# h33p/ofps

Measured on AMD Instinct MI355X. Metric: Mvectors/s, 1080p 16x16 blocks +-16 full-search SAD, higher is better.
Workload: dtype u8

## Files before the change

ofps_amd/csrc/sad.hip:

```cpp
#include "common.hpp"

#include <cstdlib>
#include <utility>

namespace {

constexpr int kWavesPerWG = 4;

constexpr int pick_stride(int min_s, int k, int ng) {
    for (int s = min_s; s < min_s + 64; ++s)
        if ((k * s) % 32 == ng % 32) return s;
    return min_s | 1;
}

template <int B, int R, int K>
struct SadCfg {
    static_assert(B % 4 == 0 && R % 4 == 0, "tile origin must stay dword aligned");
    static_assert(B * B * 255 <= 65535, "packed u16 SAD accumulators would overflow");
    static constexpr int NCAND = 2 * R + 1;
    static constexpr int NG = (NCAND + 3) / 4;
    static constexpr int NC = (NCAND + K - 1) / K;
    static constexpr int T = NG * NC;
    static constexpr int PASSES = (T + 63) / 64;
    static constexpr int BW = B / 4;
// ... 226 lines not shown
    asm volatile("" : "+v"(base));
    (strip_row<B, R, I0, RR>(acc, c, lds, base), ...);
}

#ifndef OFPS_SAD_COLKEYS
#define OFPS_SAD_COLKEYS 2
#endif
constexpr int kSadColKeys = OFPS_SAD_COLKEYS;
constexpr int kColSlotDwords = kSadColKeys == 2 ? 4 * 64 : 0;

template <int B, int R, int I0>
__device__ __forceinline__ void strip_pass(const uint32_t (&c)[B][B / 4], const uint32_t* lds, uint32_t tile_off,
                                           const uint32_t (&colk)[4], const uint32_t (&colk_pos)[4], int y0, int H, uint32_t& bkey, int& bi,
                                           uint32_t (&colmin)[4], uint32_t* amin) {
    using C = StripCfg<B, R>;
    unsigned long long acc[C::NP];
#pragma unroll
    for (int ii = 0; ii < C::NP; ++ii) acc[ii] = 0;
    constexpr int ROWS = ((I0 + C::NP < C::NCAND ? C::NP : C::NCAND - I0) + B - 1);
    strip_rows<B, R, I0>(acc, c, lds, tile_off, std::make_integer_sequence<int, ROWS>{});
#pragma unroll
    for (int ii = 0; ii < C::NP; ++ii) asm volatile("" : "+v"(acc[ii]));
    if constexpr (kSadColKeys != 0 && (C::RANK_KEY || C::COMPACT_KEY)) {
        auto low_of = [&](int ii) -> uint32_t {
            const int i = I0 + ii, dy = -R + i;
            const bool ok = i < C::NCAND && y0 + dy >= 0 && y0 + dy + B <= H;
            return ok ? (uint32_t)(C::RANK_KEY ? ((dy * dy) << 1 | (dy > 0 ? 1 : 0)) : ((dy * dy) << 6 | i)) : 0xFFFFFFFFu;
        };
        uint32_t hmask = 0xFFFF0000u;
        asm volatile("" : "+v"(hmask));
        auto keys_of = [&](int ii, uint32_t low, uint32_t (&k)[4]) {
            const uint32_t lo = (uint32_t)acc[ii], hi = (uint32_t)(acc[ii] >> 32);
            k[0] = (lo << 16) | low; k[1] = (lo & hmask) | low; k[2] = (hi << 16) | low; k[3] = (hi & hmask) | low;
        };
        if constexpr (kSadColKeys == 1) {
#pragma unroll
            for (int ii = 0; ii < C::NP; ii += 2) {
                if (I0 + ii >= C::NCAND) break;
                uint32_t ka[4], kb[4];
                keys_of(ii, low_of(ii), ka);
                if (ii + 1 < C::NP && I0 + ii + 1 < C::NCAND) {
                    keys_of(ii + 1, low_of(ii + 1), kb);
#pragma unroll
                    for (int j = 0; j < 4; ++j)
                        asm("v_min3_u32 %0, %1, %2, %3" : "=v"(colmin[j]) : "v"(colmin[j]), "v"(ka[j]), "v"(kb[j]));
                } else {
#pragma unroll
                    for (int j = 0; j < 4; ++j) colmin[j] = min(colmin[j], ka[j]);
                }
            }
        } else {
#pragma unroll
            for (int ii = 0; ii < C::NP; ++ii) {
                if (I0 + ii >= C::NCAND) break;
                uint32_t k[4];
                keys_of(ii, low_of(ii), k);
#pragma unroll
                for (int j = 0; j < 4; ++j) __hip_atomic_fetch_min(amin + 64 * j, k[j], __ATOMIC_RELAXED, __HIP_MEMORY_SCOPE_WAVEFRONT);
            }
        }
        return;
    }
#pragma unroll
    for (int ii = 0; ii < C::NP; ++ii) {
        const int i = I0 + ii;
        const int dy = -R + i;
        if (i < C::NCAND && y0 + dy >= 0 && y0 + dy + B <= H) {
            const uint32_t lo = (uint32_t)acc[ii], hi = (uint32_t)(acc[ii] >> 32);
            const uint32_t (&ck)[4] = (C::RANK_KEY && dy > 0) ? colk_pos : colk;
            const uint32_t k0 = (lo << 16) | ck[0];
            const uint32_t k1 = (lo & 0xFFFF0000u) | ck[1];
            const uint32_t k2 = (hi << 16) | ck[2];
            const uint32_t k3 = (hi & 0xFFFF0000u) | ck[3];
            if constexpr (C::RANK_KEY) {
                bkey = min(bkey, __builtin_elementwise_add_sat(min(min(k0, k1), min(k2, k3)), (uint32_t)((dy * dy) << 3)));
            } else if constexpr (C::COMPACT_KEY) {
                const uint32_t m = __builtin_elementwise_add_sat(min(min(k0, k1), min(k2, k3)), (uint32_t)((dy * dy) << 6 | i));
                bkey = min(bkey, m);
            } else {
                const uint32_t m = __builtin_elementwise_add_sat(min(min(k0, k1), min(k2, k3)), (uint32_t)(dy * dy));
                const bool lt = m < bkey;
                bkey = lt ? m : bkey;
                bi = lt ? i : bi;
            }
        }
    }
}

template <int B, int R, int... S>
__device__ __forceinline__ void strip_passes(const uint32_t (&c)[B][B / 4], const uint32_t* lds, uint32_t tile_off,
                                             const uint32_t (&colk)[4], const uint32_t (&colk_pos)[4], int y0, int H, uint32_t& bkey, int& bi,
                                             uint32_t (&colmin)[4], uint32_t* amin, std::integer_sequence<int, S...>) {
    (strip_pass<B, R, S * StripCfg<B, R>::NP>(c, lds, tile_off, colk, colk_pos, y0, H, bkey, bi, colmin, amin), ...);
}

constexpr int kStripWaves = 4;

template <int B, int R>
__device__ __forceinline__ void strip_body(const SadParams& p, int strips_per_row, int strip, uint32_t* tiles, int wave, int lane) {
    using C = StripCfg<B, R>;
    const int strips_per_pair = strips_per_row * p.nby;
    const int pair = (int)div48((unsigned)strip, p.div_spp);
    const int rem = strip - pair * strips_per_pair;
    const int by = (int)div48((unsigned)rem, p.div_spr);
    const int bx0 = (rem - by * strips_per_row) * C::NB;

    const uint8_t* __restrict__ prev = p.prev_base + (size_t)pair * p.prev_pitch;
    const uint8_t* __restrict__ cur = p.cur_base + (size_t)pair * p.cur_pitch;
    uint32_t* tile = tiles + wave * C::TILE_DWORDS;

    const int b = lane / C::NG;
    const int g = lane % C::NG;
    const int bx = bx0 + b;
    const bool blk_on = bx < p.nbx;
    const int y0 = by * B;

    uint32_t c[B][C::BW];
    {
        const int bxc = blk_on ? bx : p.nbx - 1;
        const uint8_t* cp = cur + (size_t)y0 * p.stride + bxc * B;
#pragma unroll
        for (int y = 0; y < B; ++y) {
            if constexpr (C::BW % 4 == 0) {
#pragma unroll
                for (int q4 = 0; q4 < C::BW; q4 += 4) {
                    const uint4 v = *reinterpret_cast<const uint4*>(cp + (size_t)y * p.stride + 4 * q4);
                    c[y][q4 + 0] = v.x; c[y][q4 + 1] = v.y; c[y][q4 + 2] = v.z; c[y][q4 + 3] = v.w;
                }
            } else {
#pragma unroll
                for (int q2 = 0; q2 < C::BW; q2 += 2) {
                    const uint2 v = *reinterpret_cast<const uint2*>(cp + (size_t)y * p.stride + 4 * q2);
                    c[y][q2 + 0] = v.x; c[y][q2 + 1] = v.y;
                }
            }
        }
    }

    {
        constexpr int LR = 64 / C::TILE_WG;
        constexpr int STEPS = (C::TILE_H + LR - 1) / LR;
        const int tx0 = bx0 * B - R, ty0 = y0 - R;
        const int sr = lane / C::TILE_WG, sc = lane - sr * C::TILE_WG;
        const int gx = tx0 + C::GRAN * sc;
        const bool lane_on = sr < LR && gx >= 0 && gx < p.W;
        const uint8_t* src = prev + (ptrdiff_t)(ty0 + sr) * p.stride + gx;
        uint32_t* dst = tile + sr * C::SW + C::GDW * sc;
#pragma unroll
        for (int it = 0; it < STEPS; ++it) {
            const int row = sr + it * LR;
            const bool row_in_tile = (it + 1) * LR <= C::TILE_H || row < C::TILE_H;
            if (lane_on && row_in_tile && (unsigned)(ty0 + row) < (unsigned)p.H) {
                const uint8_t* sp = src + (ptrdiff_t)(it * LR) * p.stride;
                uint32_t* dp = dst + it * LR * C::SW;
                if constexpr (C::GRAN == 16) *reinterpret_cast<uint4*>(dp) = *reinterpret_cast<const uint4*>(sp);
                else if constexpr (C::GRAN == 8) *reinterpret_cast<uint2*>(dp) = *reinterpret_cast<const uint2*>(sp);
                else *dp = *reinterpret_cast<const uint32_t*>(sp);
            }
        }
    }
    __builtin_amdgcn_fence(__ATOMIC_RELEASE, "wavefront");
    __builtin_amdgcn_wave_barrier();
    __builtin_amdgcn_fence(__ATOMIC_ACQUIRE, "wavefront");

    const int dx0 = -R + 4 * g;
    uint32_t colk[4], colk_pos[4];
#pragma unroll
    for (int j = 0; j < 4; ++j) {
        const int dx = dx0 + j;
        const int x = bx * B + dx;
        const bool v = blk_on && g < C::NGA && x >= 0 && x + B <= p.W;
        const uint32_t rank = dx0 < 0 ? 3u - j : (uint32_t)j;
        colk[j] = v ? ((uint32_t)(dx * dx) << C::KSHIFT) | (C::RANK_KEY ? rank : 0u) : 0xFFFFFFFFu;
        colk_pos[j] = v ? ((uint32_t)(dx * dx) << C::KSHIFT) | (7u - rank) : 0xFFFFFFFFu;
    }
    uint32_t bkey = 0xFFFFFFFFu;
    int bi = 0;
    uint32_t colmin[4] = {0xFFFFFFFFu, 0xFFFFFFFFu, 0xFFFFFFFFu, 0xFFFFFFFFu};
    uint32_t* amin = nullptr;
    if constexpr (kSadColKeys == 2 && (C::RANK_KEY || C::COMPACT_KEY)) {
        amin = tiles + kStripWaves * C::TILE_DWORDS + wave * kColSlotDwords + lane;
#pragma unroll
        for (int j = 0; j < 4; ++j) amin[64 * j] = 0xFFFFFFFFu;
    }
    strip_passes<B, R>(c, tiles, (uint32_t)(wave * C::TILE_DWORDS + b * C::BW + g), colk, colk_pos, y0, p.H, bkey, bi, colmin, amin,
                       std::make_integer_sequence<int, C::SPLIT>{});
    if constexpr (kSadColKeys != 0 && (C::RANK_KEY || C::COMPACT_KEY)) {
#pragma unroll
        for (int j = 0; j < 4; ++j) {
            uint32_t kc;
            if constexpr (kSadColKeys == 2) kc = __hip_atomic_load(amin + 64 * j, __ATOMIC_RELAXED, __HIP_MEMORY_SCOPE_WAVEFRONT);
            else kc = colmin[j];
            uint32_t lk;
            if constexpr (C::RANK_KEY) {
                const uint32_t x = (((kc & 0xFFFEu) << 2) + colk[j]) ^ ((kc & 1u) * 7u);
                lk = (kc & 0xFFFF0000u) | x;
            } else {
                lk = (kc & 0xFFFF0000u) | ((kc & 0xFFFFu) + colk[j]);
            }
            lk = (colk[j] == 0xFFFFFFFFu || kc == 0xFFFFFFFFu) ? 0xFFFFFFFFu : lk;
            bkey = min(bkey, lk);
        }
    }
    unsigned long long best = ~0ull;
    if (bkey != 0xFFFFFFFFu) {
        const uint32_t d2 = (bkey & 0xFFFFu) >> C::KSHIFT;
        int dx = dx0, dy;
        if constexpr (C::RANK_KEY) {
            const int code = (int)(bkey & 7u);
            const bool neg = code < 4;
            const int rank = neg ? code : 7 - code;
            dx = dx0 + (dx0 < 0 ? 3 - rank : rank);
            const int ady = (int)(__builtin_sqrtf((float)((int)d2 - dx * dx)) + 0.5f);
            dy = neg ? -ady : ady;
        } else {
            if constexpr (C::COMPACT_KEY) bi = (int)(bkey & 63u);
            dy = -R + bi;
            const int dxsq = (int)d2 - dy * dy;
#pragma unroll
            for (int j = 1; j < 4; ++j) dx = ((dx0 + j) * (dx0 + j) == dxsq) ? dx0 + j : dx;
        }
        best = ((unsigned long long)((bkey & 0xFFFF0000u) | d2) << 32) | (unsigned long long)(uint32_t)(((dy + R) << 8) | (dx + R));
    }
    uint32_t eacc[C::KE];
#pragma unroll
    for (int i = 0; i < C::KE; ++i) eacc[i] = 0;
    {
        const uint32_t* ecol = tile + b * C::BW + C::EDGE_COL;
        const int erow0 = g * C::KE;
        uint32_t nxt[C::BW];
#pragma unroll
        for (int q = 0; q < C::BW; ++q) nxt[q] = ecol[erow0 * C::SW + q];
#pragma unroll
        for (int rr = 0; rr < B + C::KE - 1; ++rr) {
            uint32_t ref[C::BW];
#pragma unroll
            for (int q = 0; q < C::BW; ++q) ref[q] = nxt[q];
            if (rr + 1 < B + C::KE - 1) {
                const int row = erow0 + rr + 1;
#pragma unroll
                for (int q = 0; q < C::BW; ++q) nxt[q] = ecol[row * C::SW + q];
            }
#pragma unroll
            for (int i = 0; i < C::KE; ++i) {
                const int y = rr - i;
                if (y >= 0 && y < B) {
#pragma unroll
                    for (int q = 0; q < C::BW; ++q) eacc[i] = __builtin_amdgcn_sad_u8(ref[q], c[y][q], eacc[i]);
                }
            }
            asm volatile("" : "+v"(eacc[0]) : : "memory");
        }
    }

    {
        const bool xok = blk_on && bx * B + R + B <= p.W;
#pragma unroll
        for (int i = 0; i < C::KE; ++i) {
            const int dy = -R + g * C::KE + i;
            const bool v = xok && dy <= R && y0 + dy >= 0 && y0 + dy + B <= p.H;
            const unsigned long long k64 =
                ((unsigned long long)((eacc[i] << 16) | (uint32_t)(R * R + dy * dy)) << 32) |
                (unsigned long long)(uint32_t)(((dy + R) << 8) | (2 * R));
            best = (v && k64 < best) ? k64 : best;
        }
    }
#pragma unroll
    for (int m = 1; m < C::NG; m <<= 1) {
        const unsigned long long o = shfl_xor_u64(best, m);
        best = o < best ? o : best;
    }
    if (blk_on && g == 0) {
        const int sad = (int)(best >> 48);
        const int dy = (int)((best >> 8) & 0xFF) - R, dx = (int)(best & 0xFF) - R;
        const size_t k = ((size_t)pair * p.nby + by) * p.nbx + bx;
        float4 e;
        e.x = (float)(bx * B + B / 2 + dx) * p.nx;
        e.y = (float)(y0 + B / 2 + dy) * p.ny;
        e.z = ((float)dx / 1.0f) * (-p.nx);
        e.w = ((float)dy / 1.0f) * (-p.ny);
        p.out_entries[k] = e;
        if (p.out_best) {
            p.out_best[3 * k + 0] = dx;
            p.out_best[3 * k + 1] = dy;
            p.out_best[3 * k + 2] = sad;
        }
    }
}

template <int B, int R>
__global__ __launch_bounds__(64 * kStripWaves, (StripCfg<B, R>::MIN_WAVES)) void sad_strip_kernel(const SadParams p, int strips_per_row,
                                                                      int total_strips) {
    using C = StripCfg<B, R>;
    __shared__ __attribute__((aligned(16))) uint32_t tiles[kStripWaves * (C::TILE_DWORDS + kColSlotDwords)];
    const int wave = __builtin_amdgcn_readfirstlane(threadIdx.x >> 6);
    const int lane = threadIdx.x & 63;
    const int per_xcd = gridDim.x / 8;
    const int lwg = (int)(blockIdx.x % 8) * per_xcd + (int)(blockIdx.x / 8);
    const int strip = lwg * kStripWaves + wave;
    if (strip >= total_strips) return;
    strip_body<B, R>(p, strips_per_row, strip, tiles, wave, lane);
}

template <int B, int R>
__global__ __launch_bounds__(64 * kStripWaves, (StripCfg<B, R>::MIN_WAVES)) void sad_strip_list_kernel(const SadParams p, int strips_per_row,
                                                                           const uint32_t* __restrict__ strip_list) {
    using C = StripCfg<B, R>;
    __shared__ __attribute__((aligned(16))) uint32_t tiles[kStripWaves * (C::TILE_DWORDS + kColSlotDwords)];
    const int wave = __builtin_amdgcn_readfirstlane(threadIdx.x >> 6);
    const int lane = threadIdx.x & 63;
    const int count = (int)strip_list[0];
#pragma unroll 1
    for (int k = (int)blockIdx.x * kStripWaves + wave; k < count; k += (int)gridDim.x * kStripWaves)
        strip_body<B, R>(p, strips_per_row, (int)strip_list[1 + k], tiles, wave, lane);
}

struct PdeCfg {
    static constexpr int B = 16, R = 16, STEP = 4, PR = B / STEP;
    using C = StripCfg<B, R>;
    static constexpr int CUR_DW = B * C::NB * C::BW;
    static constexpr int CAP = 512;
    static constexpr int WAVE_DW = C::TILE_DWORDS + 4 + CUR_DW + CAP + 2 * C::NB;
    static constexpr int OFF_CUR = C::TILE_DWORDS + 4, OFF_LIST = OFF_CUR + CUR_DW, OFF_BEST = OFF_LIST + CAP;
    static_assert(OFF_BEST % 2 == 0, "64-bit keys must be 8-byte aligned");
};

template <int RR>
__device__ __forceinline__ void pde_row(unsigned long long (&acc)[PdeCfg::C::NP], const uint32_t (&c)[PdeCfg::PR][PdeCfg::C::BW],
                                        const uint32_t* lds, uint32_t& base) {
    using C = PdeCfg::C;
    constexpr int B = PdeCfg::B, R = PdeCfg::R, STEP = PdeCfg::STEP;
    constexpr int G = StripWalk<B, R>::ROWS_PER_BASE;
    if constexpr (RR > 0 && RR % G == 0) {
        base += G * C::SW;
        asm volatile("" : "+v"(base));
    }
    unsigned long long win[C::BW];
#pragma unroll
    for (int q = 0; q < C::BW; ++q) win[q] = reinterpret_cast<const U64A4*>(lds + base + (RR % G) * C::SW + q)->v;
#pragma unroll
    for (int ii = 0; ii < C::NP; ++ii) {
        const int y = RR - ii;
        if (ii < C::NCAND && y >= 0 && y < B && y % STEP == 0) {
#pragma unroll
            for (int q = 0; q < C::BW; ++q) acc[ii] = __builtin_amdgcn_qsad_pk_u16_u8(win[q], c[y / STEP][q], acc[ii]);
        }
    }
}
template <int... RR>
__device__ __forceinline__ void pde_rows(unsigned long long (&acc)[PdeCfg::C::NP], const uint32_t (&c)[PdeCfg::PR][PdeCfg::C::BW],
                                         const uint32_t* lds, uint32_t tile_off, std::integer_sequence<int, RR...>) {
    uint32_t base = tile_off;
    asm volatile("" : "+v"(base));
    (pde_row<RR>(acc, c, lds, base), ...);
}

__device__ __forceinline__ uint32_t pde_two_rows(const uint32_t* tile, const uint32_t* curl, int bb, int dyi, int dxi, int r8) {
    using C = PdeCfg::C;
    const int sh = dxi & 3;
    uint32_t s = 0;
#pragma unroll
    for (int k = 0; k < 2; ++k) {
        const int y = 2 * r8 + k;
        const uint32_t* rp = tile + (dyi + y) * C::SW + bb * C::BW + (dxi >> 2);
        const uint32_t* cp = curl + y * (C::NB * C::BW) + bb * C::BW;
        uint32_t d[C::BW + 1];
#pragma unroll
        for (int q = 0; q <= C::BW; ++q) d[q] = rp[q];
#pragma unroll
        for (int q = 0; q < C::BW; ++q) s = __builtin_amdgcn_sad_u8(__builtin_amdgcn_alignbyte(d[q + 1], d[q], sh), cp[q], s);
    }
    return s;
}

__global__ __launch_bounds__(64 * kStripWaves, 3) void sad_pde_kernel(const SadParams p, int strips_per_row, int total_strips,
                                                                       uint32_t* __restrict__ strip_list) {
    using P = PdeCfg;
    using C = P::C;
    constexpr int B = P::B, R = P::R;
    __shared__ __attribute__((aligned(16))) uint32_t lds[kStripWaves * P::WAVE_DW];

    const int wave = __builtin_amdgcn_readfirstlane(threadIdx.x >> 6);
    const int lane = threadIdx.x & 63;
    const int per_xcd = gridDim.x / 8;
    const int lwg = (int)(blockIdx.x % 8) * per_xcd + (int)(blockIdx.x / 8);
    const int strip = lwg * kStripWaves + wave;
    if (strip >= total_strips) return;
    const int strips_per_pair = strips_per_row * p.nby;
    const int pair = strip / strips_per_pair;
    const int rem = strip - pair * strips_per_pair;
    const int by = rem / strips_per_row;
    const int bx0 = (rem - by * strips_per_row) * C::NB;
    const uint8_t* __restrict__ prev = p.prev_base + (size_t)pair * p.prev_pitch;
    const uint8_t* __restrict__ cur = p.cur_base + (size_t)pair * p.cur_pitch;
    uint32_t* tile = lds + wave * P::WAVE_DW;
    uint32_t* curl = tile + P::OFF_CUR;
    uint32_t* list = tile + P::OFF_LIST;
    unsigned long long* bestk = reinterpret_cast<unsigned long long*>(tile + P::OFF_BEST);

    const int b = lane / C::NG, g = lane % C::NG;
    const int bx = bx0 + b;
    const bool blk_on = bx < p.nbx;
    const int y0 = by * B;

    {
        const int tx0 = bx0 * B - R, ty0 = y0 - R;
        for (int idx = lane; idx < C::TILE_H * C::TILE_WG; idx += 64) {
            const int row = idx / C::TILE_WG, col = idx - row * C::TILE_WG;
            const int gx = tx0 + 16 * col, gy = ty0 + row;
            if (gy >= 0 && gy < p.H && gx >= 0 && gx < p.W)
                *reinterpret_cast<uint4*>(tile + row * C::SW + 4 * col) = *reinterpret_cast<const uint4*>(prev + (size_t)gy * p.stride + gx);
        }
#pragma unroll
        for (int k = 0; k < 2; ++k) {
            const int idx = lane + 64 * k, row = idx / C::NB, blk = idx % C::NB;
            const int bxc = min(bx0 + blk, p.nbx - 1);
            *reinterpret_cast<uint4*>(curl + row * (C::NB * C::BW) + blk * C::BW) =
                *reinterpret_cast<const uint4*>(cur + (size_t)(y0 + row) * p.stride + bxc * B);
        }
    }
    __builtin_amdgcn_fence(__ATOMIC_RELEASE, "wavefront");
    __builtin_amdgcn_wave_barrier();
    __builtin_amdgcn_fence(__ATOMIC_ACQUIRE, "wavefront");

    uint32_t c4[P::PR][C::BW];
#pragma unroll
    for (int r = 0; r < P::PR; ++r)
#pragma unroll
        for (int q = 0; q < C::BW; ++q) c4[r][q] = curl[(P::STEP * r) * (C::NB * C::BW) + b * C::BW + q];
    unsigned long long acc[C::NP];
#pragma unroll
    for (int ii = 0; ii < C::NP; ++ii) acc[ii] = 0;
    pde_rows(acc, c4, lds, (uint32_t)(wave * P::WAVE_DW + b * C::BW + g), std::make_integer_sequence<int, C::NCAND + B - 1>{});
#pragma unroll
    for (int ii = 0; ii < C::NP; ++ii) asm volatile("" : "+v"(acc[ii]));

    const int dx0 = -R + 4 * g;
    bool colv[4];
    uint32_t colk[4];
#pragma unroll
    for (int j = 0; j < 4; ++j) {
        const int x = bx * B + dx0 + j;
        colv[j] = blk_on && x >= 0 && x + B <= p.W;
        colk[j] = colv[j] ? (uint32_t)((dx0 + j) * (dx0 + j)) << C::KSHIFT : 0xFFFFFFFFu;
    }
    static_assert(C::COMPACT_KEY && C::SPLIT == 1, "written for the +-16 geometry");
    uint32_t bkey = 0xFFFFFFFFu;
#pragma unroll
    for (int i = 0; i < C::NCAND; ++i) {
        const int dy = -R + i;
        if (y0 + dy >= 0 && y0 + dy + B <= p.H) {
            const uint32_t lo = (uint32_t)acc[i], hi = (uint32_t)(acc[i] >> 32);
            const uint32_t k0 = (lo << 16) | colk[0], k1 = (lo & 0xFFFF0000u) | colk[1];
            const uint32_t k2 = (hi << 16) | colk[2], k3 = (hi & 0xFFFF0000u) | colk[3];
            bkey = min(bkey, __builtin_elementwise_add_sat(min(min(k0, k1), min(k2, k3)), (uint32_t)((dy * dy) << 6 | i)));
        }
    }
    unsigned long long pbest = ~0ull;
    if (bkey != 0xFFFFFFFFu) {
        const int bi = (int)(bkey & 63u), dy = -R + bi;
        const uint32_t d2 = (bkey & 0xFFFFu) >> C::KSHIFT;
        const int dxsq = (int)d2 - dy * dy;
        int dx = dx0;
#pragma unroll
        for (int j = 1; j < 4; ++j) dx = ((dx0 + j) * (dx0 + j) == dxsq) ? dx0 + j : dx;
        pbest = ((unsigned long long)((bkey & 0xFFFF0000u) | d2) << 32) | (unsigned long long)(uint32_t)(((dy + R) << 8) | (dx + R));
    }
    uint32_t eacc[C::KE];
    const bool xok = blk_on && bx * B + R + B <= p.W;
    {
        const uint32_t* ecol = tile + b * C::BW + C::EDGE_COL;
#pragma unroll
        for (int i = 0; i < C::KE; ++i) {
            const int dyi = min(g * C::KE + i, C::NCAND - 1);
            uint32_t sacc = 0;
#pragma unroll
            for (int r = 0; r < P::PR; ++r)
#pragma unroll
                for (int q = 0; q < C::BW; ++q) sacc = __builtin_amdgcn_sad_u8(ecol[(dyi + P::STEP * r) * C::SW + q], c4[r][q], sacc);
            eacc[i] = sacc;
            const int dy = -R + g * C::KE + i;
            const bool v = xok && dy <= R && y0 + dy >= 0 && y0 + dy + B <= p.H;
            const unsigned long long k64 = ((unsigned long long)((sacc << 16) | (uint32_t)(R * R + dy * dy)) << 32) |
                                           (unsigned long long)(uint32_t)(((dy + R) << 8) | (2 * R));
            pbest = (v && k64 < pbest) ? k64 : pbest;
        }
    }
#pragma unroll
    for (int m = 1; m < C::NG; m <<= 1) {
        const unsigned long long o = shfl_xor_u64(pbest, m);
        pbest = o < pbest ? o : pbest;
    }
    const int dy0i = blk_on ? (int)((pbest >> 8) & 0xFF) : R, dx0i = blk_on ? (int)(pbest & 0xFF) : R;
    auto key64 = [&](uint32_t sad, int dyi, int dxi) {
        const int dy = dyi - R, dx = dxi - R;
        return ((unsigned long long)((sad << 16) | (uint32_t)(dx * dx + dy * dy)) << 32) | (unsigned long long)(uint32_t)((dyi << 8) | dxi);
    };
    uint32_t U = pde_two_rows(tile, curl, b, dy0i, dx0i, g);
#pragma unroll
    for (int m = 1; m < C::NG; m <<= 1) U += __shfl_xor(U, m, 64);
    if (g == 0) bestk[b] = blk_on ? key64(U, dy0i, dx0i) : ~0ull;
    int nlist = 0;
    {
        int uj[4];
#pragma unroll
        for (int j = 0; j < 4; ++j) uj[j] = colv[j] ? (int)U : -1;
        const unsigned long long below = (1ull << lane) - 1ull;
        typedef unsigned short us2 __attribute__((ext_vector_type(2)));
        const uint32_t u1 = min(U + 1u, 0xFFFFu) * 0x10001u;
        auto any_le = [&](uint32_t v) {
            const us2 m = __builtin_elementwise_min(__builtin_bit_cast(us2, v), __builtin_bit_cast(us2, u1));
            return __builtin_bit_cast(uint32_t, m) ^ u1;
        };
#pragma unroll
        for (int i = 0; i < C::NCAND; ++i) {
            const int dy = -R + i;
            if (y0 + dy >= 0 && y0 + dy + B <= p.H) {
                const uint32_t lo = (uint32_t)acc[i], hi = (uint32_t)(acc[i] >> 32);
                if (!__ballot((any_le(lo) | any_le(hi)) != 0u)) continue;
                const int s4[4] = {(int)(lo & 0xFFFFu), (int)(lo >> 16), (int)(hi & 0xFFFFu), (int)(hi >> 16)};
#pragma unroll
                for (int j = 0; j < 4; ++j) {
                    const bool hit = s4[j] <= uj[j];
                    const unsigned long long mask = __ballot(hit);
                    if (mask) {
                        const int pos = nlist + __popcll(mask & below);
                        if (hit && pos < P::CAP) list[pos] = ((uint32_t)b << 16) | ((uint32_t)i << 8) | (uint32_t)(4 * g + j);
                        nlist += __popcll(mask);
                    }
                }
            }
        }
#pragma unroll
        for (int i = 0; i < C::KE; ++i) {
            const int dyi = g * C::KE + i, dy = dyi - R;
            const bool hit = xok && dy <= R && y0 + dy >= 0 && y0 + dy + B <= p.H && eacc[i] <= U;
            const unsigned long long mask = __ballot(hit);
            if (mask) {
                const int pos = nlist + __popcll(mask & below);
                if (hit && pos < P::CAP) list[pos] = ((uint32_t)b << 16) | ((uint32_t)dyi << 8) | (uint32_t)(2 * R);
                nlist += __popcll(mask);
            }
        }
    }
    __builtin_amdgcn_fence(__ATOMIC_RELEASE, "wavefront");
    __builtin_amdgcn_wave_barrier();
    __builtin_amdgcn_fence(__ATOMIC_ACQUIRE, "wavefront");
    const int n = nlist;
    if (n > P::CAP) {
        if (lane == 0) {
            const uint32_t pos = atomicAdd(&strip_list[0], 1u);
            strip_list[1 + pos] = (uint32_t)strip;
        }
        return;
    }
    constexpr int PER_STEP = 2 * (64 / C::NG);
    for (int base = 0; base < n; base += PER_STEP) {
        const int idx0 = base + lane / C::NG, idx1 = idx0 + 64 / C::NG;
        const uint32_t e0 = list[min(idx0, n - 1)], e1 = list[min(idx1, n - 1)];
        const int bb0 = (int)(e0 >> 16), dyi0 = (int)((e0 >> 8) & 0xFF), dxi0 = (int)(e0 & 0xFF);
        const int bb1 = (int)(e1 >> 16), dyi1 = (int)((e1 >> 8) & 0xFF), dxi1 = (int)(e1 & 0xFF);
        uint32_t s0 = pde_two_rows(tile, curl, bb0, dyi0, dxi0, g);
        uint32_t s1 = pde_two_rows(tile, curl, bb1, dyi1, dxi1, g);
#pragma unroll
        for (int m = 1; m < C::NG; m <<= 1) { s0 += __shfl_xor(s0, m, 64); s1 += __shfl_xor(s1, m, 64); }
        if (g == 0 && idx0 < n) atomicMin(&bestk[bb0], key64(s0, dyi0, dxi0));
        if (g == 0 && idx1 < n) atomicMin(&bestk[bb1], key64(s1, dyi1, dxi1));
    }
    __builtin_amdgcn_fence(__ATOMIC_RELEASE, "wavefront");
    __builtin_amdgcn_wave_barrier();
    __builtin_amdgcn_fence(__ATOMIC_ACQUIRE, "wavefront");
    if (blk_on && g == 0) write_block_result(p, pair, bx, by, B, R, bestk[b]);
}

__global__ __launch_bounds__(64) void sad_generic_kernel(const SadParams p, int B, int R) {
    const int pair = blockIdx.z, by = blockIdx.y, bx = blockIdx.x;
    const uint8_t* __restrict__ prev = p.prev_base + (size_t)pair * p.prev_pitch;
    const uint8_t* __restrict__ cur = p.cur_base + (size_t)pair * p.cur_pitch;
    const int x0 = bx * B, y0 = by * B, n = 2 * R + 1;
    unsigned long long best = ~0ull;
    for (int cand = threadIdx.x; cand < n * n; cand += 64) {
        const int dy = cand / n - R, dx = cand % n - R;
        if (x0 + dx < 0 || x0 + dx + B > p.W || y0 + dy < 0 || y0 + dy + B > p.H) continue;
        uint32_t sad = 0;
        for (int y = 0; y < B; ++y) {
            const uint8_t* cr = cur + (size_t)(y0 + y) * p.stride + x0;
            const uint8_t* pr = prev + (size_t)(y0 + dy + y) * p.stride + x0 + dx;
            for (int x = 0; x < B; ++x) {
                const int d = (int)cr[x] - (int)pr[x];
                sad += (uint32_t)(d < 0 ? -d : d);
            }
        }
        const unsigned long long key = ((unsigned long long)sad << 32) | ((unsigned long long)(dx * dx + dy * dy) << 16) |
                                       (unsigned long long)(((dy + R) << 8) | (dx + R));
        best = key < best ? key : best;
    }
#pragma unroll
    for (int m = 32; m >= 1; m >>= 1) {
        const unsigned long long o = shfl_xor_u64(best, m);
        best = o < best ? o : best;
    }
    if (threadIdx.x == 0) {
        const int sad = (int)(best >> 32);
        const int dy = (int)((best >> 8) & 0xFF) - R, dx = (int)(best & 0xFF) - R;
        const size_t k = ((size_t)pair * p.nby + by) * p.nbx + bx;
        float4 e;
        e.x = (float)(x0 + B / 2 + dx) * p.nx;
        e.y = (float)(y0 + B / 2 + dy) * p.ny;
        e.z = ((float)dx / 1.0f) * (-p.nx);
        e.w = ((float)dy / 1.0f) * (-p.ny);
        p.out_entries[k] = e;
        if (p.out_best) {
            p.out_best[3 * k + 0] = dx;
            p.out_best[3 * k + 1] = dy;
            p.out_best[3 * k + 2] = sad;
        }
    }
}

template <int B, int R, int K>
void launch_qsad(const SadParams& p, int pairs, hipStream_t s) {
    dim3 grid((p.nbx + kWavesPerWG - 1) / kWavesPerWG, p.nby, pairs);
    hipLaunchKernelGGL((sad_qsad_kernel<B, R, K>), grid, dim3(256), 0, s, p);
}

inline void strip_div_magic(SadParams& q, int strips_per_row) {
    q.div_spp = div_magic48((unsigned)strips_per_row * (unsigned)q.nby);
    q.div_spr = div_magic48((unsigned)strips_per_row);
}

template <int B, int R>
void launch_strip(const SadParams& p, int pairs, hipStream_t s) {
    using C = StripCfg<B, R>;
    const int strips_per_row = (p.nbx + C::NB - 1) / C::NB;
    const int total = strips_per_row * p.nby * pairs;
    const int nwg = ((total + kStripWaves - 1) / kStripWaves + 7) / 8 * 8;
    SadParams q = p;
    strip_div_magic(q, strips_per_row);
    hipLaunchKernelGGL((sad_strip_kernel<B, R>), dim3(nwg), dim3(64 * kStripWaves), 0, s, q, strips_per_row, total);
}

int launch_pde_16_16(ofps_hip_ctx* ctx, const SadParams& p, int pairs, hipStream_t s) {
    using C = StripCfg<16, 16>;
    const int strips_per_row = (p.nbx + C::NB - 1) / C::NB;
    const int total = strips_per_row * p.nby * pairs;
    auto* strip_list = static_cast<uint32_t*>(ofps::scratch(ctx, ofps::S_SAD_LIST, (size_t)(total + 1) * sizeof(uint32_t)));
    if (!strip_list) return OFPS_HIP_ENOMEM;
    OFPS_HIP_TRY(ctx, hipMemsetAsync(strip_list, 0, sizeof(uint32_t), s));
    const int nwg = ((total + kStripWaves - 1) / kStripWaves + 7) / 8 * 8;
    hipLaunchKernelGGL(sad_pde_kernel, dim3(nwg), dim3(64 * kStripWaves), 0, s, p, strips_per_row, total, strip_list);
    const int nwg_ind = nwg < 8 * ctx->num_cus ? nwg : 8 * ctx->num_cus;
    SadParams q = p;
    strip_div_magic(q, strips_per_row);
    hipLaunchKernelGGL((sad_strip_list_kernel<16, 16>), dim3(nwg_ind), dim3(64 * kStripWaves), 0, s, q, strips_per_row,
                       (const uint32_t*)strip_list);
    return OFPS_HIP_OK;
}

}

extern "C" {

size_t ofps_hip_sad_block_count(int W, int H, int block) {
    if (W <= 0 || H <= 0 || block <= 0) return 0;
    return (size_t)(W / block) * (size_t)(H / block);
}

}

namespace ofps {
int sad_pairs_device(ofps_hip_ctx* ctx, const uint8_t* prev_base, size_t prev_pitch, const uint8_t* cur_base,
                     size_t cur_pitch, int pairs, int W, int H, int stride, int block, int range, void* d_out_entries,
                     void* d_out_best) {
    OFPS_REQUIRE(ctx, W > 0 && H > 0 && stride >= W, "sad_flow: bad geometry W=%d H=%d stride=%d", W, H, stride);
    OFPS_REQUIRE(ctx, stride % 4 == 0 && ((uintptr_t)prev_base % 4) == 0 && ((uintptr_t)cur_base % 4) == 0 &&
                          prev_pitch % 4 == 0 && cur_pitch % 4 == 0,
                 "sad_flow: rows must be 4-byte aligned (stride=%d)", stride);
    OFPS_REQUIRE(ctx, block >= 1 && block <= 64 && range >= 0 && range <= 64,
                 "sad_flow: block=%d range=%d outside [1,64]/[0,64]", block, range);
    SadParams p{};
    p.prev_base = prev_base; p.cur_base = cur_base;
    p.prev_pitch = prev_pitch; p.cur_pitch = cur_pitch;
    p.W = W; p.H = H; p.stride = stride;
    p.nbx = W / block; p.nby = H / block;
    p.nx = 1.0f / (float)W; p.ny = 1.0f / (float)H;
    p.out_entries = static_cast<float4*>(d_out_entries);
    p.out_best = static_cast<int*>(d_out_best);
    if (p.nbx == 0 || p.nby == 0 || pairs <= 0) return OFPS_HIP_OK;
    OFPS_REQUIRE(ctx, pairs <= 65535 && p.nby <= 65535, "sad_flow: grid too large");
    OFPS_HIP_TRY(ctx, hipSetDevice(ctx->device));
    const bool qpel = ctx->opt.sad_motion_scale == 4;
    if (qpel && !p.out_best) {
        p.out_best = static_cast<int*>(ofps::scratch(ctx, ofps::S_SAD_QBEST, (size_t)pairs * p.nbx * p.nby * 3 * sizeof(int)));
        if (!p.out_best) return OFPS_HIP_ENOMEM;
    }
    hipStream_t s = ctx->stream;
    const int key = block * 1000 + range;
    const bool force_block = ctx->opt.sad_force_block != 0;
    const bool strip_ok = !force_block && stride % 16 == 0 && ((uintptr_t)prev_base % 16) == 0 &&
                          ((uintptr_t)cur_base % 16) == 0 && prev_pitch % 16 == 0 && cur_pitch % 16 == 0 &&
                          (long long)p.nbx * p.nby * pairs < (1ll << 28) && (long long)p.nbx * p.nby < (1ll << 20);
    switch (key) {
        case 16016:
            if (strip_ok && ctx->sad_mode == OFPS_HIP_SAD_PRUNED) {
                const int rc = launch_pde_16_16(ctx, p, pairs, s);
                if (rc != OFPS_HIP_OK) return rc;
            } else if (strip_ok) launch_strip<16, 16>(p, pairs, s);
            else launch_qsad<16, 16, 5>(p, pairs, s);
            break;
        case 16008:
            if (strip_ok) launch_strip<16, 8>(p, pairs, s); else launch_qsad<16, 8, 3>(p, pairs, s);
            break;
        case 16032:
            if (strip_ok) launch_strip<16, 32>(p, pairs, s); else launch_qsad<16, 32, 5>(p, pairs, s);
            break;
        case 8032:
            if (strip_ok) launch_strip<8, 32>(p, pairs, s); else launch_qsad<8, 32, 5>(p, pairs, s);
            break;
        case 8016:
            if (strip_ok) launch_strip<8, 16>(p, pairs, s); else launch_qsad<8, 16, 5>(p, pairs, s);
            break;
        case 8008:
            if (strip_ok) launch_strip<8, 8>(p, pairs, s); else launch_qsad<8, 8, 3>(p, pairs, s);
            break;
#define OFPS_STRIP_CASE(BB, RR)                                         \
        case BB * 1000 + RR:                                            \
            if (strip_ok) { launch_strip<BB, RR>(p, pairs, s); break; } \
            [[fallthrough]];
        OFPS_STRIP_CASE(16, 12) OFPS_STRIP_CASE(16, 20) OFPS_STRIP_CASE(16, 24) OFPS_STRIP_CASE(16, 28)
        OFPS_STRIP_CASE(8, 12) OFPS_STRIP_CASE(8, 20) OFPS_STRIP_CASE(8, 24) OFPS_STRIP_CASE(8, 28)
#undef OFPS_STRIP_CASE
        default: {
            dim3 grid(p.nbx, p.nby, pairs);
            hipLaunchKernelGGL(sad_generic_kernel, grid, dim3(64), 0, s, p, block, range);
        }
    }
    OFPS_HIP_TRY(ctx, hipGetLastError());
    if (qpel)
        return ofps::sad_qpel_refine_device(ctx, prev_base, prev_pitch, cur_base, cur_pitch, pairs, W, H, stride, block, range, d_out_entries,
                                            p.out_best, d_out_best);
    return OFPS_HIP_OK;
}
}

extern "C" {

int ofps_hip_sad_flow_dev(ofps_hip_ctx* ctx, const void* d_frames, int n_frames, int W, int H, int stride,
                          size_t frame_pitch, int ref_mode, int block, int range, void* d_out_entries,
                          void* d_out_best) {
    if (!ctx) return OFPS_HIP_EINVAL;
    OFPS_REQUIRE(ctx, d_frames && d_out_entries, "sad_flow: null device pointer");
    OFPS_REQUIRE(ctx, n_frames >= 2, "sad_flow: need at least 2 frames (got %d)", n_frames);
    OFPS_REQUIRE(ctx, frame_pitch >= (size_t)stride * (size_t)H, "sad_flow: frame_pitch smaller than a frame");
    OFPS_REQUIRE(ctx, ref_mode == 0 || ref_mode == 1, "sad_flow: ref_mode must be 0 or 1");
    const auto* f = static_cast<const uint8_t*>(d_frames);
    return ofps::sad_pairs_device(ctx, f, ref_mode ? 0 : frame_pitch, f + frame_pitch, frame_pitch, n_frames - 1, W, H, stride,
                                  block, range, d_out_entries, d_out_best);
}

int ofps_hip_sad_flow(ofps_hip_ctx* ctx, const uint8_t* prev, const uint8_t* cur, int W, int H, int stride,
                      int block, int range, float* out_entries, int32_t* out_best, size_t* n_out) {
    if (!ctx) return OFPS_HIP_EINVAL;
    OFPS_REQUIRE(ctx, prev && cur && out_entries, "sad_flow: null host pointer");
    OFPS_REQUIRE(ctx, W > 0 && H > 0 && stride >= W && block >= 1, "sad_flow: bad geometry");
    OFPS_HIP_TRY(ctx, hipSetDevice(ctx->device));
    const int dstride = (W + 63) & ~63;
    const size_t pitch = (size_t)dstride * H;
    const size_t nblk = ofps_hip_sad_block_count(W, H, block);
    auto* d_frames = static_cast<uint8_t*>(ofps::scratch(ctx, ofps::S_FRAMES, 2 * pitch));
    auto* d_ent = static_cast<float*>(ofps::scratch(ctx, ofps::S_ENTRIES, nblk * 4 * sizeof(float)));
    auto* d_best = static_cast<int32_t*>(ofps::scratch(ctx, ofps::S_BEST, nblk * 3 * sizeof(int32_t)));
    if (!d_frames || !d_ent || !d_best) return OFPS_HIP_ENOMEM;
    OFPS_HIP_TRY(ctx, ofps::upload_rows(d_frames, dstride, prev, stride, W, H, ctx->stream));
    OFPS_HIP_TRY(ctx, ofps::upload_rows(d_frames + pitch, dstride, cur, stride, W, H, ctx->stream));
    int rc = ofps_hip_sad_flow_dev(ctx, d_frames, 2, W, H, dstride, pitch, 0, block, range, d_ent, d_best);
    if (rc != OFPS_HIP_OK) return rc;
    if (nblk) {
        OFPS_HIP_TRY(ctx, hipMemcpyAsync(out_entries, d_ent, nblk * 4 * sizeof(float), hipMemcpyDeviceToHost, ctx->stream));
        if (out_best)
            OFPS_HIP_TRY(ctx, hipMemcpyAsync(out_best, d_best, nblk * 3 * sizeof(int32_t), hipMemcpyDeviceToHost, ctx->stream));
    }
    OFPS_HIP_TRY(ctx, hipStreamSynchronize(ctx->stream));
    if (n_out) *n_out = nblk;
    return OFPS_HIP_OK;
}

int ofps_hip_sad_pruned_overflow_strips(ofps_hip_ctx* ctx, uint32_t* count) {
    if (!ctx || !count) return OFPS_HIP_EINVAL;
    *count = 0;
    auto& sc = ctx->scratch[ofps::S_SAD_LIST];
    if (!sc.p) return OFPS_HIP_OK;
    OFPS_HIP_TRY(ctx, hipSetDevice(ctx->device));
    OFPS_HIP_TRY(ctx, hipStreamSynchronize(ctx->stream));
    OFPS_HIP_TRY(ctx, hipMemcpy(count, sc.p, sizeof(uint32_t), hipMemcpyDeviceToHost));
    return OFPS_HIP_OK;
}

int ofps_hip_set_sad_mode(ofps_hip_ctx* ctx, int mode) {
    if (!ctx) return OFPS_HIP_EINVAL;
    OFPS_REQUIRE(ctx, mode == OFPS_HIP_SAD_EXHAUSTIVE || mode == OFPS_HIP_SAD_PRUNED, "set_sad_mode: unknown mode %d", mode);
    ctx->sad_mode = mode;
    return OFPS_HIP_OK;
}

}
```

Baseline: 517.7.

## Finish dense PDE strips in-kernel and refine survivors per 4-column quad

The partial-distance-elimination kernel no longer hands strips with too many surviving candidates to a second full-search launch. It finishes them in place by accumulating the remaining 12 rows into the existing qsad accumulators and edge sums. For sparse strips, survivors are now packed as 16-bit quad entries (block, column group, row), and each lane refines one quad with qsad over all 16 rows instead of two rows per candidate per lane. This removes the second kernel launch and its redundant recomputation of partial sums, and makes the refinement loop more uniform. In exchange the dense path raises register pressure, and a global atomic counter is now incremented for each dense strip.

New measurement: 516.3. Within noise of the previous version (-0.3%).

```diff
diff --git a/ofps_amd/csrc/sad.hip b/ofps_amd/csrc/sad.hip
--- a/ofps_amd/csrc/sad.hip
+++ b/ofps_amd/csrc/sad.hip
@@ -552,31 +552,21 @@
     strip_body<B, R>(p, strips_per_row, strip, tiles, wave, lane);
 }
 
-template <int B, int R>
-__global__ __launch_bounds__(64 * kStripWaves, (StripCfg<B, R>::MIN_WAVES)) void sad_strip_list_kernel(const SadParams p, int strips_per_row,
-                                                                           const uint32_t* __restrict__ strip_list) {
-    using C = StripCfg<B, R>;
-    __shared__ __attribute__((aligned(16))) uint32_t tiles[kStripWaves * (C::TILE_DWORDS + kColSlotDwords)];
-    const int wave = __builtin_amdgcn_readfirstlane(threadIdx.x >> 6);
-    const int lane = threadIdx.x & 63;
-    const int count = (int)strip_list[0];
-#pragma unroll 1
-    for (int k = (int)blockIdx.x * kStripWaves + wave; k < count; k += (int)gridDim.x * kStripWaves)
-        strip_body<B, R>(p, strips_per_row, (int)strip_list[1 + k], tiles, wave, lane);
-}
-
 struct PdeCfg {
     static constexpr int B = 16, R = 16, STEP = 4, PR = B / STEP;
     using C = StripCfg<B, R>;
     static constexpr int CUR_DW = B * C::NB * C::BW;
-    static constexpr int CAP = 512;
-    static constexpr int WAVE_DW = C::TILE_DWORDS + 4 + CUR_DW + CAP + 2 * C::NB;
-    static constexpr int OFF_CUR = C::TILE_DWORDS + 4, OFF_LIST = OFF_CUR + CUR_DW, OFF_BEST = OFF_LIST + CAP;
+    static constexpr int LIST_DW = 512;
+    static constexpr int DENSE_QUADS = 1024;
+    static_assert(DENSE_QUADS <= 2 * LIST_DW, "every strip below the threshold must fit the list");
+    static constexpr int WAVE_DW = C::TILE_DWORDS + 4 + CUR_DW + LIST_DW + 2 * C::NB;
+    static constexpr int OFF_CUR = C::TILE_DWORDS + 4, OFF_LIST = OFF_CUR + CUR_DW, OFF_BEST = OFF_LIST + LIST_DW;
     static_assert(OFF_BEST % 2 == 0, "64-bit keys must be 8-byte aligned");
+    static_assert(OFF_CUR % 4 == 0 && WAVE_DW % 4 == 0, "rows of the current frame are read 16 bytes at a time");
 };
 
-template <int RR>
-__device__ __forceinline__ void pde_row(unsigned long long (&acc)[PdeCfg::C::NP], const uint32_t (&c)[PdeCfg::PR][PdeCfg::C::BW],
+template <bool REST, int RR, int NROWS>
+__device__ __forceinline__ void pde_row(unsigned long long (&acc)[PdeCfg::C::NP], const uint32_t (&c)[NROWS][PdeCfg::C::BW],
                                         const uint32_t* lds, uint32_t& base) {
     using C = PdeCfg::C;
     constexpr int B = PdeCfg::B, R = PdeCfg::R, STEP = PdeCfg::STEP;
@@ -591,18 +581,45 @@
 #pragma unroll
     for (int ii = 0; ii < C::NP; ++ii) {
         const int y = RR - ii;
-        if (ii < C::NCAND && y >= 0 && y < B && y % STEP == 0) {
-#pragma unroll
-            for (int q = 0; q < C::BW; ++q) acc[ii] = __builtin_amdgcn_qsad_pk_u16_u8(win[q], c[y / STEP][q], acc[ii]);
-        }
-    }
-}
-template <int... RR>
-__device__ __forceinline__ void pde_rows(unsigned long long (&acc)[PdeCfg::C::NP], const uint32_t (&c)[PdeCfg::PR][PdeCfg::C::BW],
+        if (ii < C::NCAND && y >= 0 && y < B && (y % STEP != 0) == REST) {
+            const int cy = REST ? y - y / STEP - 1 : y / STEP;
+#pragma unroll
+            for (int q = 0; q < C::BW; ++q) acc[ii] = __builtin_amdgcn_qsad_pk_u16_u8(win[q], c[cy][q], acc[ii]);
+        }
+    }
+}
+template <bool REST, int NROWS, int... RR>
+__device__ __forceinline__ void pde_rows(unsigned long long (&acc)[PdeCfg::C::NP], const uint32_t (&c)[NROWS][PdeCfg::C::BW],
                                          const uint32_t* lds, uint32_t tile_off, std::integer_sequence<int, RR...>) {
     uint32_t base = tile_off;
     asm volatile("" : "+v"(base));
-    (pde_row<RR>(acc, c, lds, base), ...);
+    (pde_row<REST, RR>(acc, c, lds, base), ...);
+}
+
+__device__ __forceinline__ unsigned long long pde_lane_best(const unsigned long long (&acc)[PdeCfg::C::NP], const uint32_t (&colk)[4],
+                                                            int dx0, int y0, int H) {
+    using C = PdeCfg::C;
+    constexpr int B = PdeCfg::B, R = PdeCfg::R;
+    static_assert(C::COMPACT_KEY && C::SPLIT == 1, "written for the +-16 geometry");
+    uint32_t bkey = 0xFFFFFFFFu;
+#pragma unroll
+    for (int i = 0; i < C::NCAND; ++i) {
+        const int dy = -R + i;
+        if (y0 + dy >= 0 && y0 + dy + B <= H) {
+            const uint32_t lo = (uint32_t)acc[i], hi = (uint32_t)(acc[i] >> 32);
+            const uint32_t k0 = (lo << 16) | colk[0], k1 = (lo & 0xFFFF0000u) | colk[1];
+            const uint32_t k2 = (hi << 16) | colk[2], k3 = (hi & 0xFFFF0000u) | colk[3];
+            bkey = min(bkey, __builtin_elementwise_add_sat(min(min(k0, k1), min(k2, k3)), (uint32_t)((dy * dy) << 6 | i)));
+        }
+    }
+    if (bkey == 0xFFFFFFFFu) return ~0ull;
+    const int bi = (int)(bkey & 63u), dy = -R + bi;
+    const uint32_t d2 = (bkey & 0xFFFFu) >> C::KSHIFT;
+    const int dxsq = (int)d2 - dy * dy;
+    int dx = dx0;
+#pragma unroll
+    for (int j = 1; j < 4; ++j) dx = ((dx0 + j) * (dx0 + j) == dxsq) ? dx0 + j : dx;
+    return ((unsigned long long)((bkey & 0xFFFF0000u) | d2) << 32) | (unsigned long long)(uint32_t)(((dy + R) << 8) | (dx + R));
 }
 
 __device__ __forceinline__ uint32_t pde_two_rows(const uint32_t* tile, const uint32_t* curl, int bb, int dyi, int dxi, int r8) {
@@ -624,7 +641,7 @@
 }
 
 __global__ __launch_bounds__(64 * kStripWaves, 3) void sad_pde_kernel(const SadParams p, int strips_per_row, int total_strips,
-                                                                       uint32_t* __restrict__ strip_list) {
+                                                                       uint32_t* __restrict__ dense_strips) {
     using P = PdeCfg;
     using C = P::C;
     constexpr int B = P::B, R = P::R;
@@ -645,7 +662,7 @@
     const uint8_t* __restrict__ cur = p.cur_base + (size_t)pair * p.cur_pitch;
     uint32_t* tile = lds + wave * P::WAVE_DW;
     uint32_t* curl = tile + P::OFF_CUR;
-    uint32_t* list = tile + P::OFF_LIST;
+    unsigned short* list = reinterpret_cast<unsigned short*>(tile + P::OFF_LIST);
     unsigned long long* bestk = reinterpret_cast<unsigned long long*>(tile + P::OFF_BEST);
 
     const int b = lane / C::NG, g = lane % C::NG;
@@ -673,6 +690,7 @@
     __builtin_amdgcn_wave_barrier();
     __builtin_amdgcn_fence(__ATOMIC_ACQUIRE, "wavefront");
 
+    const uint32_t tile_off = (uint32_t)(wave * P::WAVE_DW + b * C::BW + g);
     uint32_t c4[P::PR][C::BW];
 #pragma unroll
     for (int r = 0; r < P::PR; ++r)
@@ -681,7 +699,7 @@
     unsigned long long acc[C::NP];
 #pragma unroll
     for (int ii = 0; ii < C::NP; ++ii) acc[ii] = 0;
-    pde_rows(acc, c4, lds, (uint32_t)(wave * P::WAVE_DW + b * C::BW + g), std::make_integer_sequence<int, C::NCAND + B - 1>{});
+    pde_rows<false>(acc, c4, lds, tile_off, std::make_integer_sequence<int, C::NCAND + B - 1>{});
 #pragma unroll
     for (int ii = 0; ii < C::NP; ++ii) asm volatile("" : "+v"(acc[ii]));
 
@@ -694,47 +712,27 @@
         colv[j] = blk_on && x >= 0 && x + B <= p.W;
         colk[j] = colv[j] ? (uint32_t)((dx0 + j) * (dx0 + j)) << C::KSHIFT : 0xFFFFFFFFu;
     }
-    static_assert(C::COMPACT_KEY && C::SPLIT == 1, "written for the +-16 geometry");
-    uint32_t bkey = 0xFFFFFFFFu;
-#pragma unroll
-    for (int i = 0; i < C::NCAND; ++i) {
-        const int dy = -R + i;
-        if (y0 + dy >= 0 && y0 + dy + B <= p.H) {
-            const uint32_t lo = (uint32_t)acc[i], hi = (uint32_t)(acc[i] >> 32);
-            const uint32_t k0 = (lo << 16) | colk[0], k1 = (lo & 0xFFFF0000u) | colk[1];
-            const uint32_t k2 = (hi << 16) | colk[2], k3 = (hi & 0xFFFF0000u) | colk[3];
-            bkey = min(bkey, __builtin_elementwise_add_sat(min(min(k0, k1), min(k2, k3)), (uint32_t)((dy * dy) << 6 | i)));
-        }
-    }
-    unsigned long long pbest = ~0ull;
-    if (bkey != 0xFFFFFFFFu) {
-        const int bi = (int)(bkey & 63u), dy = -R + bi;
-        const uint32_t d2 = (bkey & 0xFFFFu) >> C::KSHIFT;
-        const int dxsq = (int)d2 - dy * dy;
-        int dx = dx0;
-#pragma unroll
-        for (int j = 1; j < 4; ++j) dx = ((dx0 + j) * (dx0 + j) == dxsq) ? dx0 + j : dx;
-        pbest = ((unsigned long long)((bkey & 0xFFFF0000u) | d2) << 32) | (unsigned long long)(uint32_t)(((dy + R) << 8) | (dx + R));
-    }
+    unsigned long long pbest = pde_lane_best(acc, colk, dx0, y0, p.H);
     uint32_t eacc[C::KE];
     const bool xok = blk_on && bx * B + R + B <= p.W;
-    {
-        const uint32_t* ecol = tile + b * C::BW + C::EDGE_COL;
-#pragma unroll
-        for (int i = 0; i < C::KE; ++i) {
-            const int dyi = min(g * C::KE + i, C::NCAND - 1);
-            uint32_t sacc = 0;
-#pragma unroll
-            for (int r = 0; r < P::PR; ++r)
-#pragma unroll
-                for (int q = 0; q < C::BW; ++q) sacc = __builtin_amdgcn_sad_u8(ecol[(dyi + P::STEP * r) * C::SW + q], c4[r][q], sacc);
-            eacc[i] = sacc;
-            const int dy = -R + g * C::KE + i;
-            const bool v = xok && dy <= R && y0 + dy >= 0 && y0 + dy + B <= p.H;
-            const unsigned long long k64 = ((unsigned long long)((sacc << 16) | (uint32_t)(R * R + dy * dy)) << 32) |
-                                           (unsigned long long)(uint32_t)(((dy + R) << 8) | (2 * R));
-            pbest = (v && k64 < pbest) ? k64 : pbest;
-        }
+    auto edge_key = [&](uint32_t sum, int dy) {
+        return ((unsigned long long)((sum << 16) | (uint32_t)(R * R + dy * dy)) << 32) | (unsigned long long)(uint32_t)(((dy + R) << 8) | (2 * R));
+    };
+    auto edge_on = [&](int dy) { return xok && dy <= R && y0 + dy >= 0 && y0 + dy + B <= p.H; };
+    const uint32_t* ecol = tile + b * C::BW + C::EDGE_COL;
+#pragma unroll
+    for (int i = 0; i < C::KE; ++i) {
+        const int dyi = min(g * C::KE + i, C::NCAND - 1);
+        uint32_t sacc = 0;
+#pragma unroll
+        for (int r = 0; r < P::PR; ++r)
+#pragma unroll
+            for (int q = 0; q < C::BW; ++q) sacc = __builtin_amdgcn_sad_u8(ecol[(dyi + P::STEP * r) * C::SW + q], c4[r][q], sacc);
+        asm volatile("" : "+v"(sacc) : : "memory");
+        eacc[i] = sacc;
+        const int dy = -R + g * C::KE + i;
+        const unsigned long long k64 = edge_key(sacc, dy);
+        pbest = (edge_on(dy) && k64 < pbest) ? k64 : pbest;
     }
 #pragma unroll
     for (int m = 1; m < C::NG; m <<= 1) {
@@ -749,73 +747,120 @@
     uint32_t U = pde_two_rows(tile, curl, b, dy0i, dx0i, g);
 #pragma unroll
     for (int m = 1; m < C::NG; m <<= 1) U += __shfl_xor(U, m, 64);
-    if (g == 0) bestk[b] = blk_on ? key64(U, dy0i, dx0i) : ~0ull;
-    int nlist = 0;
+    int nq = 0;
     {
-        int uj[4];
-#pragma unroll
-        for (int j = 0; j < 4; ++j) uj[j] = colv[j] ? (int)U : -1;
         const unsigned long long below = (1ull << lane) - 1ull;
+        const bool lane_on = colv[0] | colv[1] | colv[2] | colv[3];
         typedef unsigned short us2 __attribute__((ext_vector_type(2)));
         const uint32_t u1 = min(U + 1u, 0xFFFFu) * 0x10001u;
         auto any_le = [&](uint32_t v) {
             const us2 m = __builtin_elementwise_min(__builtin_bit_cast(us2, v), __builtin_bit_cast(us2, u1));
             return __builtin_bit_cast(uint32_t, m) ^ u1;
         };
+        auto append = [&](bool hit, uint32_t entry) {
+            const unsigned long long mask = __ballot(hit);
+            if (mask) {
+                const int pos = nq + __popcll(mask & below);
+                if (hit && pos < 2 * P::LIST_DW) list[pos] = (unsigned short)entry;
+                nq += __popcll(mask);
+            }
+        };
+#pragma unroll
+        for (int i = 0; i < C::KE; ++i) {
+            const int dyi = g * C::KE + i;
+            append(edge_on(dyi - R) && eacc[i] <= U, ((uint32_t)b << 10) | ((uint32_t)C::NG << 6) | (uint32_t)dyi);
+        }
+        const uint32_t ebase = ((uint32_t)b << 10) | ((uint32_t)g << 6);
 #pragma unroll
         for (int i = 0; i < C::NCAND; ++i) {
             const int dy = -R + i;
-            if (y0 + dy >= 0 && y0 + dy + B <= p.H) {
-                const uint32_t lo = (uint32_t)acc[i], hi = (uint32_t)(acc[i] >> 32);
-                if (!__ballot((any_le(lo) | any_le(hi)) != 0u)) continue;
-                const int s4[4] = {(int)(lo & 0xFFFFu), (int)(lo >> 16), (int)(hi & 0xFFFFu), (int)(hi >> 16)};
-#pragma unroll
-                for (int j = 0; j < 4; ++j) {
-                    const bool hit = s4[j] <= uj[j];
-                    const unsigned long long mask = __ballot(hit);
-                    if (mask) {
-                        const int pos = nlist + __popcll(mask & below);
-                        if (hit && pos < P::CAP) list[pos] = ((uint32_t)b << 16) | ((uint32_t)i << 8) | (uint32_t)(4 * g + j);
-                        nlist += __popcll(mask);
+            if (y0 + dy >= 0 && y0 + dy + B <= p.H)
+                append(lane_on && (any_le((uint32_t)acc[i]) | any_le((uint32_t)(acc[i] >> 32))) != 0u, ebase | (uint32_t)i);
+        }
+    }
+    if (nq > P::DENSE_QUADS) {
+        if (lane == 0) atomicAdd(dense_strips, 1u);
+        uint32_t cr[B - P::PR][C::BW];
+#pragma unroll
+        for (int y = 0; y < B; ++y)
+            if (y % P::STEP != 0) {
+                const uint4 v = *reinterpret_cast<const uint4*>(curl + y * (C::NB * C::BW) + b * C::BW);
+                uint32_t (&d)[C::BW] = cr[y - y / P::STEP - 1];
+                d[0] = v.x; d[1] = v.y; d[2] = v.z; d[3] = v.w;
+            }
+        pde_rows<true>(acc, cr, lds, tile_off, std::make_integer_sequence<int, C::NCAND + B - 1>{});
+#pragma unroll
+        for (int ii = 0; ii < C::NP; ++ii) asm volatile("" : "+v"(acc[ii]));
+        unsigned long long best = pde_lane_best(acc, colk, dx0, y0, p.H);
+        {
+            const int erow0 = g * C::KE;
+            uint32_t nxt[C::BW];
+#pragma unroll
+            for (int q = 0; q < C::BW; ++q) nxt[q] = ecol[erow0 * C::SW + q];
+#pragma unroll
+            for (int rr = 0; rr < B + C::KE - 1; ++rr) {
+                uint32_t ref[C::BW];
+#pragma unroll
+                for (int q = 0; q < C::BW; ++q) ref[q] = nxt[q];
+                if (rr + 1 < B + C::KE - 1) {
+                    const int row = erow0 + rr + 1;
+#pragma unroll
+                    for (int q = 0; q < C::BW; ++q) nxt[q] = ecol[row * C::SW + q];
+                }
+#pragma unroll
+                for (int i = 0; i < C::KE; ++i) {
+                    const int y = rr - i;
+                    if (y >= 0 && y < B && y % P::STEP != 0) {
+#pragma unroll
+                        for (int q = 0; q < C::BW; ++q) eacc[i] = __builtin_amdgcn_sad_u8(ref[q], cr[y - y / P::STEP - 1][q], eacc[i]);
                     }
                 }
+                asm volatile("" : "+v"(eacc[0]) : : "memory");
             }
         }
 #pragma unroll
         for (int i = 0; i < C::KE; ++i) {
-            const int dyi = g * C::KE + i, dy = dyi - R;
-            const bool hit = xok && dy <= R && y0 + dy >= 0 && y0 + dy + B <= p.H && eacc[i] <= U;
-            const unsigned long long mask = __ballot(hit);
-            if (mask) {
-                const int pos = nlist + __popcll(mask & below);
-                if (hit && pos < P::CAP) list[pos] = ((uint32_t)b << 16) | ((uint32_t)dyi << 8) | (uint32_t)(2 * R);
-                nlist += __popcll(mask);
-            }
-        }
-    }
+            const int dy = -R + g * C::KE + i;
+            const unsigned long long k64 = edge_key(eacc[i], dy);
+            best = (edge_on(dy) && k64 < best) ? k64 : best;
+        }
+#pragma unroll
+        for (int m = 1; m < C::NG; m <<= 1) {
+            const unsigned long long o = shfl_xor_u64(best, m);
+            best = o < best ? o : best;
+        }
+        if (blk_on && g == 0) write_block_result(p, pair, bx, by, B, R, best);
+        return;
+    }
+    if (g == 0) bestk[b] = blk_on ? key64(U, dy0i, dx0i) : ~0ull;
     __builtin_amdgcn_fence(__ATOMIC_RELEASE, "wavefront");
     __builtin_amdgcn_wave_barrier();
     __builtin_amdgcn_fence(__ATOMIC_ACQUIRE, "wavefront");
-    const int n = nlist;
-    if (n > P::CAP) {
-        if (lane == 0) {
-            const uint32_t pos = atomicAdd(&strip_list[0], 1u);
-            strip_list[1 + pos] = (uint32_t)strip;
-        }
-        return;
-    }
-    constexpr int PER_STEP = 2 * (64 / C::NG);
-    for (int base = 0; base < n; base += PER_STEP) {
-        const int idx0 = base + lane / C::NG, idx1 = idx0 + 64 / C::NG;
-        const uint32_t e0 = list[min(idx0, n - 1)], e1 = list[min(idx1, n - 1)];
-        const int bb0 = (int)(e0 >> 16), dyi0 = (int)((e0 >> 8) & 0xFF), dxi0 = (int)(e0 & 0xFF);
-        const int bb1 = (int)(e1 >> 16), dyi1 = (int)((e1 >> 8) & 0xFF), dxi1 = (int)(e1 & 0xFF);
-        uint32_t s0 = pde_two_rows(tile, curl, bb0, dyi0, dxi0, g);
-        uint32_t s1 = pde_two_rows(tile, curl, bb1, dyi1, dxi1, g);
-#pragma unroll
-        for (int m = 1; m < C::NG; m <<= 1) { s0 += __shfl_xor(s0, m, 64); s1 += __shfl_xor(s1, m, 64); }
-        if (g == 0 && idx0 < n) atomicMin(&bestk[bb0], key64(s0, dyi0, dxi0));
-        if (g == 0 && idx1 < n) atomicMin(&bestk[bb1], key64(s1, dyi1, dxi1));
+#pragma unroll 1
+    for (int base = 0; base < nq; base += 64) {
+        const int idx = base + lane;
+        const uint32_t e = list[min(idx, nq - 1)];
+        const int bb = (int)(e >> 10), gg = (int)((e >> 6) & 15u), dyi = (int)(e & 63u);
+        const uint32_t* wp = tile + dyi * C::SW + bb * C::BW + gg;
+        const uint32_t* cp = curl + bb * C::BW;
+        unsigned long long a = 0;
+#pragma unroll
+        for (int y = 0; y < B; ++y) {
+            const uint4 cv = *reinterpret_cast<const uint4*>(cp + y * (C::NB * C::BW));
+            const uint32_t cw[C::BW] = {cv.x, cv.y, cv.z, cv.w};
+#pragma unroll
+            for (int q = 0; q < C::BW; ++q) a = __builtin_amdgcn_qsad_pk_u16_u8(reinterpret_cast<const U64A4*>(wp + y * C::SW + q)->v, cw[q], a);
+        }
+        const uint32_t s4[4] = {(uint32_t)a & 0xFFFFu, ((uint32_t)a >> 16), (uint32_t)(a >> 32) & 0xFFFFu, (uint32_t)(a >> 48)};
+        const int x0 = (bx0 + bb) * B - R + 4 * gg;
+        unsigned long long k = ~0ull;
+#pragma unroll
+        for (int j = 0; j < 4; ++j) {
+            const bool v = idx < nq && bx0 + bb < p.nbx && 4 * gg + j <= 2 * R && x0 + j >= 0 && x0 + j + B <= p.W;
+            const unsigned long long kj = key64(s4[j], dyi, 4 * gg + j);
+            k = (v && kj < k) ? kj : k;
+        }
+        if (k != ~0ull) atomicMin(&bestk[bb], k);
     }
     __builtin_amdgcn_fence(__ATOMIC_RELEASE, "wavefront");
     __builtin_amdgcn_wave_barrier();
@@ -894,16 +939,11 @@
     using C = StripCfg<16, 16>;
     const int strips_per_row = (p.nbx + C::NB - 1) / C::NB;
     const int total = strips_per_row * p.nby * pairs;
-    auto* strip_list = static_cast<uint32_t*>(ofps::scratch(ctx, ofps::S_SAD_LIST, (size_t)(total + 1) * sizeof(uint32_t)));
-    if (!strip_list) return OFPS_HIP_ENOMEM;
-    OFPS_HIP_TRY(ctx, hipMemsetAsync(strip_list, 0, sizeof(uint32_t), s));
+    auto* dense_strips = static_cast<uint32_t*>(ofps::scratch(ctx, ofps::S_SAD_LIST, sizeof(uint32_t)));
+    if (!dense_strips) return OFPS_HIP_ENOMEM;
+    OFPS_HIP_TRY(ctx, hipMemsetAsync(dense_strips, 0, sizeof(uint32_t), s));
     const int nwg = ((total + kStripWaves - 1) / kStripWaves + 7) / 8 * 8;
-    hipLaunchKernelGGL(sad_pde_kernel, dim3(nwg), dim3(64 * kStripWaves), 0, s, p, strips_per_row, total, strip_list);
-    const int nwg_ind = nwg < 8 * ctx->num_cus ? nwg : 8 * ctx->num_cus;
-    SadParams q = p;
-    strip_div_magic(q, strips_per_row);
-    hipLaunchKernelGGL((sad_strip_list_kernel<16, 16>), dim3(nwg_ind), dim3(64 * kStripWaves), 0, s, q, strips_per_row,
-                       (const uint32_t*)strip_list);
+    hipLaunchKernelGGL(sad_pde_kernel, dim3(nwg), dim3(64 * kStripWaves), 0, s, p, strips_per_row, total, dense_strips);
     return OFPS_HIP_OK;
 }
 
```
